# rare-resilience-ai/Osteosarcoma_DiffusionModel

Measured on AMD Instinct MI355X. Metric: synthetic patients/sec (full T-step reverse sample), higher is better.
Workload: dtype f32; 1 GPU; reverse sampling of conditional patients, T=1000, D=2000 (50 mut + 1900 expr + 50 pathway), hidden [256,512,256], 3 scenario conditions (BASELINE config 3); patients_per_gpu=100000, T=1000, parallelism=patients sharded over 1 GPU(s), no collective, sampler=chain, chunk_rows=65536, streams=2, graph=True

## Files before the change

### osteosarcoma_diffusionmodel_amd/csrc/chain.h

```cpp
#pragma once
#include "gemm_glds.h"
#include "epilogues.h"
#include "xpose.h"
#include "launch.h"

namespace osd {

constexpr int CHAIN_MAX_LAYERS = 24;
enum : int { CK_INPUT = 0, CK_GN32 = 1, CK_GN64 = 2, CK_POST = 3 };
enum : unsigned { CHAIN_OK = 0, CHAIN_TIMEOUT = 1, CHAIN_ABORT = 2 };

struct ChainLayer {
  const float* A; int lda;
  int K, K0;
  int F;
  int in0, ld0, in1, ld1;
  int out, ldo;
  int kind;
  const float* bias; const float* gamma; const float* beta;
};

struct ChainArgs {
  ChainLayer L[CHAIN_MAX_LAYERS];
  int n_layers;
  float* ws; long long ws_stride;
  float* x; int D;
  int n, n_tiles;
  int t_first, n_steps;
  unsigned base_done;
  const float* cproj; int ldc;
  const float* temb; int ldt;
  const float* coef;
  const float* z; int ldzz; long long z_step_stride; int z_t_first;
  uint64_t seed; uint32_t row_offset;
  float* mut_mask; int mutation_dim;
  unsigned* progress;
  unsigned* status;
  unsigned* queue;
  unsigned* cu_arrivals;
  int stagger;
  unsigned long long spin_budget;
  unsigned long long* stamps;
};

typedef __attribute__((address_space(1))) unsigned gu32;

__device__ __forceinline__ unsigned ld_relaxed_agent(const unsigned* p) {
  return __hip_atomic_load(p, __ATOMIC_RELAXED, __HIP_MEMORY_SCOPE_AGENT);
}
__device__ __forceinline__ void st_relaxed_agent(unsigned* p, unsigned v) {
  __hip_atomic_store(p, v, __ATOMIC_RELAXED, __HIP_MEMORY_SCOPE_AGENT);
}

__device__ __forceinline__ bool chain_wait(const unsigned* word, unsigned want, unsigned* status, unsigned long long budget, int lane) {
  if ((unsigned)__builtin_amdgcn_readfirstlane((int)ld_relaxed_agent(word)) >= want) return true;
  const unsigned long long t0 = __builtin_amdgcn_s_memrealtime();
  for (;;) {
    __builtin_amdgcn_s_sleep(32);
    if ((unsigned)__builtin_amdgcn_readfirstlane((int)ld_relaxed_agent(word)) >= want) return true;
    if ((unsigned)__builtin_amdgcn_readfirstlane((int)ld_relaxed_agent(status)) != CHAIN_OK) return false;
    if (__builtin_amdgcn_s_memrealtime() - t0 > budget) {
      if (lane == 0) st_relaxed_agent(status, CHAIN_TIMEOUT);
      return false;
    }
  }
}

constexpr int CHAIN_PRM_FLOATS = 512;

template <int NPB>
struct XposeRowsOut {
  const WaveXpose<NPB>& xp; float* out; int ldo;
  __device__ __forceinline__ void put(int fb, int pb, int q, int l31, int h, float4 v) const { (void)fb; xp.put(pb, q, l31, h, v); }
  __device__ __forceinline__ void flush(int fb, int lane) const { xp.template store_rows<false>(out + 32 * fb, ldo, lane, 0, 0); }
};
template <int NPB>
struct XposeRowsIn {
  const WaveXpose<NPB>& xp; const float* src; int ld;
  __device__ __forceinline__ void load(int fb, int lane) const { xp.template load_rows<false>(src + 32 * fb, ld, lane, 0, 0); }
  __device__ __forceinline__ float4 get(int fb, int pb, int q, int l31, int h) const { (void)fb; return xp.get(pb, q, l31, h); }
};

template <int GW, int NFB, int NPB, int PS, class Out>
__device__ __forceinline__ void chain_gn_silu(f32x16 (&acc)[NFB][NPB], const float* __restrict__ prm, int fl, const Out& o, int lane,
                                              unsigned long long* ts = nullptr) {
  static_assert(GW >= 8 && NFB * 32 >= GW, "wave must own whole groups");
  constexpr int RPG = GW / 2;
  constexpr int NG = NFB * 16 / RPG;
  const int l31 = lane & 31, h = lane >> 5;
#pragma unroll
  for (int fb = 0; fb < NFB; ++fb)
#pragma unroll
    for (int q = 0; q < 4; ++q) {
      const float4 bv = *reinterpret_cast<const float4*>(prm + fl + 32 * fb + 8 * q + 4 * h);
#pragma unroll
      for (int pb = 0; pb < NPB; ++pb) {
        acc[fb][pb][4 * q] += bv.x; acc[fb][pb][4 * q + 1] += bv.y;
        acc[fb][pb][4 * q + 2] += bv.z; acc[fb][pb][4 * q + 3] += bv.w;
      }
    }
  if (ts) { asm volatile("s_waitcnt vmcnt(0) lgkmcnt(0)" ::: "memory"); ts[0] = __builtin_amdgcn_s_memtime(); }
  float mean[NPB][NG], rstd[NPB][NG];
#pragma unroll
  for (int pb = 0; pb < NPB; ++pb)
#pragma unroll
    for (int g = 0; g < NG; ++g) {
      float s = 0.f;
#pragma unroll
      for (int j = 0; j < RPG; ++j) { const int Li = g * RPG + j; s += acc[Li / 16][pb][Li % 16]; }
      s += swap_halves(s);
      const float m = s * (1.0f / GW);
      float qs = 0.f;
#pragma unroll
      for (int j = 0; j < RPG; ++j) { const int Li = g * RPG + j; const float d = acc[Li / 16][pb][Li % 16] - m; qs = fmaf(d, d, qs); }
      qs += swap_halves(qs);
      mean[pb][g] = m;
      rstd[pb][g] = 1.0f / sqrtf(qs * (1.0f / GW) + GN_EPS);
    }
  if (ts) { asm volatile("s_nop 0" ::: "memory"); ts[1] = __builtin_amdgcn_s_memtime(); ts[2] = ts[1]; }
#pragma unroll
  for (int fb = 0; fb < NFB; ++fb) {
#pragma unroll
    for (int q = 0; q < 4; ++q) {
      const int f = fl + 32 * fb + 8 * q + 4 * h;
      const float4 gv = *reinterpret_cast<const float4*>(prm + PS + f);
      const float4 bev = *reinterpret_cast<const float4*>(prm + 2 * PS + f);
      const int g = (fb * 16 + 4 * q) / RPG;
#pragma unroll
      for (int pb = 0; pb < NPB; ++pb) {
        const float m = mean[pb][g], r = rstd[pb][g];
        float4 y;
        y.x = silu_f(fmaf((acc[fb][pb][4 * q] - m) * r, gv.x, bev.x));
        y.y = silu_f(fmaf((acc[fb][pb][4 * q + 1] - m) * r, gv.y, bev.y));
        y.z = silu_f(fmaf((acc[fb][pb][4 * q + 2] - m) * r, gv.z, bev.z));
        y.w = silu_f(fmaf((acc[fb][pb][4 * q + 3] - m) * r, gv.w, bev.w));
        o.put(fb, pb, q, l31, h, y);
      }
    }
    o.flush(fb, lane);
  }
}

template <int NFB, int NPB, int PS, class In, class Out>
__device__ __forceinline__ void chain_input(f32x16 (&acc)[NFB][NPB], const float* __restrict__ prm, int fl, const In& in, const Out& o, int lane) {
  const int l31 = lane & 31, h = lane >> 5;
#pragma unroll
  for (int fb = 0; fb < NFB; ++fb) {
    in.load(fb, lane);
#pragma unroll
    for (int q = 0; q < 4; ++q) {
      const int f = fl + 32 * fb + 8 * q + 4 * h;
      const float4 bv = *reinterpret_cast<const float4*>(prm + f);
      const float4 tv = *reinterpret_cast<const float4*>(prm + PS + f);
#pragma unroll
      for (int pb = 0; pb < NPB; ++pb) {
        const float4 cv = in.get(fb, pb, q, l31, h);
        float4 v;
        v.x = ((acc[fb][pb][4 * q] + bv.x) + tv.x) + cv.x;
        v.y = ((acc[fb][pb][4 * q + 1] + bv.y) + tv.y) + cv.y;
        v.z = ((acc[fb][pb][4 * q + 2] + bv.z) + tv.z) + cv.z;
        v.w = ((acc[fb][pb][4 * q + 3] + bv.w) + tv.w) + cv.w;
        o.put(fb, pb, q, l31, h, v);
      }
    }
    o.flush(fb, lane);
  }
}

#ifndef OSD_EXP
#define OSD_EXP 0
#endif
template <int NFB, int NPB, bool PRE = false, bool GUARD = true>
__device__ __forceinline__ void chain_posterior(f32x16 (&acc)[NFB][NPB], const float* __restrict__ prm, int fl, float* __restrict__ x, int ldx,
                                                int prow, int pcol, float cA, float cB, float cC, int t, const float* __restrict__ zrow, int ldzz,
                                                uint64_t seed, uint32_t row_id0, int f_glob, float* __restrict__ mut_mask, int mutation_dim,
                                                const WaveXpose<NPB>& xp, int lane, float4 (*pre)[4 * NPB] = nullptr) {
  const int l31 = lane & 31, h = lane >> 5;
  if (prow <= 0) return;
  const bool do_mask = t == 0 && mut_mask != nullptr;
#pragma unroll
  for (int fb = 0; fb < NFB; ++fb) {
    const int cols = pcol - 32 * fb;
    if (GUARD && cols <= 0) break;
    if constexpr (PRE) {
      if (!(OSD_EXP & 2)) {
        xp.commit_rows(*pre, lane);
        if (fb + 1 < NFB && cols - 32 > 0) xp.template issue_rows<GUARD>(*pre, x + 32 * (fb + 1), ldx, lane, prow, cols - 32);
      }
    } else {
      xp.template load_rows<GUARD>(x + 32 * fb, ldx, lane, prow, cols);
    }
#pragma unroll
    for (int pb = 0; pb < NPB; ++pb) {
      const int p = 32 * pb + l31;
      const int pc = (!GUARD || p < prow) ? p : prow - 1;
#pragma unroll
      for (int q = 0; q < 4; ++q) {
        const int fo = 32 * fb + 8 * q + 4 * h;
        const float4 bv = *reinterpret_cast<const float4*>(prm + fl + fo);
        const float e[4] = {acc[fb][pb][4 * q] + bv.x, acc[fb][pb][4 * q + 1] + bv.y, acc[fb][pb][4 * q + 2] + bv.z, acc[fb][pb][4 * q + 3] + bv.w};
        const float4 xq = xp.get(pb, q, l31, h);
        const float xv[4] = {xq.x, xq.y, xq.z, xq.w};
        float4 zz = make_float4(0.f, 0.f, 0.f, 0.f);
        if (t > 0 && cC != 0.f) {
          if (zrow) {
            const int fc = (!GUARD || fo < pcol - 4) ? fo : pcol - 4;
            zz = ldg4(zrow + (size_t)pc * ldzz + fc);
          } else if (!(OSD_EXP & 1)) {
            zz = randn4(seed, row_id0 + (uint32_t)p, (uint32_t)((f_glob + fo) >> 2), (uint32_t)t, TAG_POSTERIOR);
          }
        }
        const float zv[4] = {zz.x, zz.y, zz.z, zz.w};
        float o[4];
#pragma unroll
        for (int r = 0; r < 4; ++r) o[r] = fmaf(cA, xv[r], fmaf(cB, e[r], cC * zv[r]));
        if (do_mask && p < prow && fo < pcol && f_glob + fo < mutation_dim) {
          float* mrow = mut_mask + (size_t)p * mutation_dim;
#pragma unroll
          for (int r = 0; r < 4; ++r)
            if (f_glob + fo + r < mutation_dim) stg1(mrow + f_glob + fo + r, (o[r] > 0.5f) ? 1.0f : 0.0f);
        }
        xp.put(pb, q, l31, h, make_float4(o[0], o[1], o[2], o[3]));
      }
    }
    if (!(OSD_EXP & 4)) xp.template store_rows<GUARD>(x + 32 * fb, ldx, lane, prow, cols);
  }
}

#ifndef CHAIN_EPI_PRIO
#define CHAIN_EPI_PRIO 0
#endif
#ifndef CHAIN_BP
#define CHAIN_BP 128
#endif
#if CHAIN_BP == 128
typedef Tile<128, 128, 64, 64> ChainTile;
constexpr int CHAIN_WPS = 2;
#else
typedef Tile<128, 64, 64, 32> ChainTile;
constexpr int CHAIN_WPS = 3;
#endif
#ifdef OSD_DIAG
constexpr int CHAIN_KCNT = 12;
constexpr int CHAIN_STAMP_FLOATS = 2 * 4 * CHAIN_KCNT;
#else
constexpr int CHAIN_KCNT = 10;
constexpr int CHAIN_STAMP_FLOATS = 80;
#endif
constexpr int CHAIN_PRM_OFF = 2 * (ChainTile::BF * BK + ChainTile::BP * BK) + 4 + CHAIN_STAMP_FLOATS;
constexpr int CHAIN_LDS_BYTES = (CHAIN_PRM_OFF + 2 * CHAIN_PRM_FLOATS) * 4;
static_assert(CHAIN_PRM_OFF % 4 == 0, "parameter blocks are read as float4");

template <bool STAMP>
__global__ __launch_bounds__(NTHREADS, CHAIN_WPS) void chain_kernel(const ChainArgs* __restrict__ gp) {
  const ChainArgs& a = *gp;
  typedef ChainTile T;
  typedef GldsTile<T> G;
  static_assert(T::BF == 128 && T::BP % 32 == 0, "staging below assumes a 128-row weight image");
  constexpr int NW = NTHREADS / 64;
  constexpr int NPW = 16 / NW;
  constexpr int NPWB = T::BP / 8 / NW;
  constexpr int PROWS = 8 * NW;
  constexpr unsigned PBYTES = 1024u * NW;
  extern __shared__ __attribute__((aligned(16))) float smem[];
  float* As0 = smem;
  float* As1 = smem + G::A_ELEMS;
  float* Bs0 = smem + 2 * G::A_ELEMS;
  float* Bs1 = smem + 2 * G::A_ELEMS + G::B_ELEMS;
  volatile int& s_flag = *reinterpret_cast<volatile int*>(smem + 2 * (G::A_ELEMS + G::B_ELEMS));

  const int tid = threadIdx.x;
  const int lane = tid & 63;
  const int wave = __builtin_amdgcn_readfirstlane(tid >> 6);
  const int wf = (wave / T::NWP) * T::WF;
  const int wp = (wave % T::NWP) * T::WP;

  float* const ws = a.ws + (long long)blockIdx.x * a.ws_stride;
  WaveXpose<T::NPB> xp;
  {
    const int xo = wave * (T::NPB * 1024);
    xp.buf = xo < G::A_ELEMS ? As1 + xo : Bs1 + (xo - G::A_ELEMS);
  }
  float* const prm_base = smem + CHAIN_PRM_OFF;
  int pcur = 0;

  if (a.cu_arrivals && a.stagger > 0) {
    if (wave == 0) {
      const unsigned hw = __builtin_amdgcn_s_getreg(0xF804);
      const unsigned xcc = __builtin_amdgcn_s_getreg(0xF814) & 7;
      const unsigned key = (xcc << 8) | ((hw >> 8) & 0xFF);
      unsigned r = 0;
      if (lane == 0) r = atomicAdd(a.cu_arrivals + key, 1u);
      s_flag = __builtin_amdgcn_readfirstlane((int)(r & 1u));
    }
    __syncthreads();
    const int late = __builtin_amdgcn_readfirstlane(s_flag);
    __syncthreads();
    if (late) {
      const unsigned long long t0 = __builtin_amdgcn_s_memtime();
      while (__builtin_amdgcn_s_memtime() - t0 < (unsigned long long)a.stagger) __builtin_amdgcn_s_sleep(16);
    }
  }

  unsigned long long c_dep = 0, c_pro = 0, c_k = 0, c_epi = 0, c_units = 0;
  unsigned long long* const kcnt = reinterpret_cast<unsigned long long*>(smem + 2 * (G::A_ELEMS + G::B_ELEMS) + 4);
  if constexpr (STAMP) {
    if (tid < 4 * CHAIN_KCNT) kcnt[tid] = 0;
    __syncthreads();
  }
  const unsigned long long c_start = STAMP ? __builtin_amdgcn_s_memtime() : 0;
  const long long n_units = (long long)a.n_tiles * a.n_steps;
  int c_iter = 0;
  (void)c_iter;
  for (;;) {
    const unsigned long long td0 = STAMP ? __builtin_amdgcn_s_memtime() : 0;
#ifdef CHAIN_STATIC_UNITS
    static_assert(true, "");
    const long long u = (long long)blockIdx.x + (long long)c_iter * gridDim.x;
    ++c_iter;
#else
    if (wave == 0) {
      unsigned nu = 0;
      if (lane == 0) nu = atomicAdd(a.queue, 1u);
      s_flag = __builtin_amdgcn_readfirstlane((int)nu);
    }
    __syncthreads();
    const long long u = (unsigned)__builtin_amdgcn_readfirstlane(s_flag);
    __syncthreads();
#endif
    if (u >= n_units) break;
    const int tile = (int)(u % a.n_tiles);
    const int si = (int)(u / a.n_tiles);
    const int t = a.t_first - si;
    const int p0 = tile * T::BP;
    const int P = (a.n - p0 < T::BP) ? a.n - p0 : T::BP;

    if (wave == 0) {
      bool ok = (unsigned)__builtin_amdgcn_readfirstlane((int)ld_relaxed_agent(a.status)) == CHAIN_OK;
      if (ok && si > 0) {
        ok = chain_wait(a.progress + tile, a.base_done + (unsigned)si, a.status, a.spin_budget, lane);
        if (ok) __builtin_amdgcn_fence(__ATOMIC_ACQUIRE, "agent");
      }
      s_flag = ok ? 1 : 0;
      asm volatile("s_waitcnt vmcnt(0) lgkmcnt(0)" ::: "memory");
    }
    __syncthreads();
    const int go = __builtin_amdgcn_readfirstlane(s_flag);
    if (!go) return;
    if constexpr (STAMP) { c_dep += __builtin_amdgcn_s_memtime() - td0; ++c_units; }

    auto first_stage = [&](const ChainLayer& Lr, int f0n, bool do_a, bool do_b, int pb) {
      struct { const float* A; int lda, F, in0, ld0, K0, K; } Ln{Lr.A, Lr.lda, Lr.F, Lr.in0, Lr.ld0, Lr.K0, Lr.K};
      if (do_a && wave < 2) {
        const int kind = Lr.kind;
        const float* src = Lr.bias;
        if (wave == 1) src = Lr.beta;
        else if (lane >= 32) src = kind == CK_INPUT ? a.temb + (size_t)t * a.ldt : (kind == CK_POST ? Lr.bias : Lr.gamma);
        if (wave == 0 || (kind != CK_INPUT && kind != CK_POST)) {
          int f = f0n + 4 * (lane & 31);
          f = f < Ln.F - 4 ? f : Ln.F - 4;
          glds16(src + f, __builtin_amdgcn_readfirstlane(lds_addr(prm_base + pb * CHAIN_PRM_FLOATS) + (unsigned)wave * 1024u));
        }
      }
      const float* const xrows = a.x + (size_t)p0 * a.D;
      int ln = lane;
      asm volatile("" : "+v"(ln));
      const int r0 = wave * 8 + (ln >> 3);
      const int k4 = 4 * ((ln & 7) ^ ((r0 >> 1) & 7));
      const unsigned la = __builtin_amdgcn_readfirstlane(lds_addr(As0) + (unsigned)wave * 1024u);
      const unsigned lb = __builtin_amdgcn_readfirstlane(lds_addr(Bs0) + (unsigned)wave * 1024u);
      if (do_a) {
#pragma unroll
        for (int j = 0; j < NPW; ++j) {
          int rg = f0n + r0 + PROWS * j;
          rg = rg < Ln.F ? rg : Ln.F - 1;
          glds16(Ln.A + (size_t)rg * Ln.lda + k4, __builtin_amdgcn_readfirstlane(la + (unsigned)j * PBYTES));
        }
      }
      if (do_b) {
        const bool from_x = Ln.in0 < 0;
        const float* bb = from_x ? xrows : ws + Ln.in0;
        const int rows = from_x ? P : T::BP;
        const int kend = Ln.K0 < Ln.K ? Ln.K0 : Ln.K;
        const int k = k4 < kend - 4 ? k4 : kend - 4;
#pragma unroll
        for (int j = 0; j < NPWB; ++j) {
          int rg = r0 + PROWS * j;
          rg = rg < rows ? rg : rows - 1;
          glds16(bb + (size_t)rg * Ln.ld0 + k, __builtin_amdgcn_readfirstlane(lb + (unsigned)j * PBYTES));
        }
      }
    };
    unsigned long long tt0 = STAMP ? __builtin_amdgcn_s_memtime() : 0;
    first_stage(a.L[0], 0, true, true, pcur);
    asm volatile("s_waitcnt vmcnt(0)" ::: "memory");
    __syncthreads();

    for (int l = 0; l < a.n_layers; ++l) {
      const ChainLayer& L = a.L[l];
      const gfloat_ptr LA = uniform_ptr(L.A);
      const int Llda = L.lda, LK0 = L.K0, Lld0 = L.ld0, Lld1 = L.ld1;
      const int F = L.F, K = L.K;
      const float* const B0g = (L.in0 < 0) ? a.x + (size_t)p0 * a.D : ws + L.in0;
      const float* const B1g = ws + L.in1;
      const gfloat_ptr B0 = uniform_ptr(B0g), B1 = uniform_ptr(B1g);
      const int rowsB = (L.in0 < 0) ? P : T::BP;
      const int nk = (K + BK - 1) / BK;
      const int nft = (F + T::BF - 1) / T::BF;
      for (int ft = 0; ft < nft; ++ft) {
        const int f0 = ft * T::BF;
        int ln = lane;
        asm volatile("" : "+v"(ln));
        const int l31 = ln & 31, h = ln >> 5;
        int st_row[NPW], st_k4[NPW];
#pragma unroll
        for (int j = 0; j < NPW; ++j) {
          st_row[j] = (j * NW + wave) * 8 + (ln >> 3);
          st_k4[j] = 4 * ((ln & 7) ^ ((st_row[j] >> 1) & 7));
        }
        int a_rd[T::NFB], a_sw[T::NFB], b_rd[T::NPB], b_sw[T::NPB];
#pragma unroll
        for (int fb = 0; fb < T::NFB; ++fb) { const int R = wf + 32 * fb + l31; a_rd[fb] = R * BK; a_sw[fb] = h ^ ((R >> 1) & 7); }
#pragma unroll
        for (int pb = 0; pb < T::NPB; ++pb) { const int R = wp + 32 * pb + l31; b_rd[pb] = R * BK; b_sw[pb] = h ^ ((R >> 1) & 7); }
        unsigned offA[NPW], offB[NPWB];
#pragma unroll
        for (int j = 0; j < NPW; ++j) {
          int rg = f0 + st_row[j];
          rg = rg < F ? rg : F - 1;
          offA[j] = (unsigned)(rg * Llda + st_k4[j]) * 4u;
        }
#pragma unroll
        for (int j = 0; j < NPWB; ++j) {
          int rb = st_row[j];
          rb = rb < rowsB ? rb : rowsB - 1;
          offB[j] = (unsigned)(rb * Lld0 + st_k4[j]) * 4u;
        }
        int b_panel = 0;
        auto b_offsets_for = [&](int k0) {
          const int want = k0 < LK0 ? 0 : 1;
          if (want != b_panel) {
            b_panel = want;
            const int ld = want ? Lld1 : Lld0;
#pragma unroll
            for (int j = 0; j < NPWB; ++j) {
              int rb = st_row[j];
              rb = rb < rowsB ? rb : rowsB - 1;
              offB[j] = (unsigned)(rb * ld + st_k4[j]) * 4u;
            }
          }
        };
        struct StageCtx { gfloat_ptr sa, sb; unsigned la, lb; int k0; bool tail; };
        auto stage_begin = [&](int k0, float* As, float* Bs) {
          b_offsets_for(k0);
          const bool first = k0 < LK0;
          const int kend = first ? (LK0 < K ? LK0 : K) : K - LK0;
          const int kl = first ? k0 : k0 - LK0;
          StageCtx c;
          c.sa = LA + __builtin_amdgcn_readfirstlane(k0);
          c.sb = (first ? B0 : B1) + __builtin_amdgcn_readfirstlane(kl);
          c.la = __builtin_amdgcn_readfirstlane(lds_addr(As) + (unsigned)wave * 1024u);
          c.lb = __builtin_amdgcn_readfirstlane(lds_addr(Bs) + (unsigned)wave * 1024u);
          c.k0 = k0;
          c.tail = kl + BK > kend;
          return c;
        };
        auto piece = [&](const StageCtx& c, int j) {
          if (j < NPW) glds16s(c.sa, offA[j], __builtin_amdgcn_readfirstlane(c.la + (unsigned)j * PBYTES));
          else glds16s(c.sb, offB[j - NPW], __builtin_amdgcn_readfirstlane(c.lb + (unsigned)(j - NPW) * PBYTES));
        };
        auto stage_tail = [&](const StageCtx& c) {
#pragma unroll
          for (int j = 0; j < NPW; ++j) piece(c, j);
          const bool first = c.k0 < LK0;
          const int kend = first ? (LK0 < K ? LK0 : K) : K - LK0;
          const int kl = first ? c.k0 : c.k0 - LK0;
          const float* bb = first ? B0g : B1g;
          const int ld = first ? Lld0 : Lld1;
#pragma unroll
          for (int jb = 0; jb < NPWB; ++jb) {
            int k = kl + st_k4[jb];
            k = k < kend - 4 ? k : kend - 4;
            int rg = st_row[jb];
            rg = rg < rowsB ? rg : rowsB - 1;
            glds16(bb + (size_t)rg * ld + k, __builtin_amdgcn_readfirstlane(c.lb + (unsigned)jb * PBYTES));
          }
        };
        const unsigned long long tt1 = STAMP ? __builtin_amdgcn_s_memtime() : 0;

        unsigned long long c_kw = 0, c_kb = 0;
        (void)c_kw; (void)c_kb;
        f32x16 acc[T::NFB][T::NPB];
#pragma unroll
        for (int i = 0; i < T::NFB; ++i)
#pragma unroll
          for (int j = 0; j < T::NPB; ++j)
#pragma unroll
            for (int r = 0; r < 16; ++r) acc[i][j][r] = 0.f;

        float fa0[T::NFB][4], fb0[T::NPB][4], fa1[T::NFB][4], fb1[T::NPB][4];
        auto frags = [&](const float* Ac, const float* Bc, int i, float (&fa)[T::NFB][4], float (&fb)[T::NPB][4]) {
#pragma unroll
          for (int fb_ = 0; fb_ < T::NFB; ++fb_) {
            const float4 tq = *reinterpret_cast<const float4*>(&Ac[a_rd[fb_] + 4 * (a_sw[fb_] ^ (2 * i))]);
            fa[fb_][0] = tq.x; fa[fb_][1] = tq.y; fa[fb_][2] = tq.z; fa[fb_][3] = tq.w;
          }
#pragma unroll
          for (int pb = 0; pb < T::NPB; ++pb) {
            const float4 tq = *reinterpret_cast<const float4*>(&Bc[b_rd[pb] + 4 * (b_sw[pb] ^ (2 * i))]);
            fb[pb][0] = tq.x; fb[pb][1] = tq.y; fb[pb][2] = tq.z; fb[pb][3] = tq.w;
          }
        };
        auto quarter = [&](const float (&fa)[T::NFB][4], const float (&fb)[T::NPB][4]) {
#pragma unroll
          for (int e = 0; e < 4; ++e)
#pragma unroll
            for (int fb_ = 0; fb_ < T::NFB; ++fb_)
#pragma unroll
              for (int pb = 0; pb < T::NPB; ++pb)
                acc[fb_][pb] = __builtin_amdgcn_mfma_f32_32x32x2f32(fa[fb_][e], fb[pb][e], acc[fb_][pb], 0, 0, 0);
        };
        __builtin_amdgcn_sched_barrier(0);
        if (nk > 1) {
          const StageCtx c = stage_begin(BK, As1, Bs1);
          if (c.tail) stage_tail(c);
          else {
#pragma unroll
            for (int j = 0; j < NPW + NPWB; ++j) piece(c, j);
          }
        }
        frags(As0, Bs0, 0, fa0, fb0);
        __builtin_amdgcn_sched_barrier(0);
        for (int kt = 0; kt < nk; ++kt) {
          float* Ac = (kt & 1) ? As1 : As0;
          float* Bc = (kt & 1) ? Bs1 : Bs0;
          const float* An = (kt & 1) ? As0 : As1;
          const float* Bn = (kt & 1) ? Bs0 : Bs1;
          frags(Ac, Bc, 1, fa1, fb1);
          quarter(fa0, fb0);
          frags(Ac, Bc, 2, fa0, fb0);
          quarter(fa1, fb1);
          frags(Ac, Bc, 3, fa1, fb1);
          const bool ahead = kt + 2 < nk;
          StageCtx c{};
          if (ahead) c = stage_begin((kt + 2) * BK, Ac, Bc);
          const bool whole = ahead && !c.tail;
          quarter(fa0, fb0);
          __builtin_amdgcn_sched_barrier(0);
          const unsigned long long tw0 = STAMP ? __builtin_amdgcn_s_memtime() : 0;
          asm volatile("s_waitcnt vmcnt(0)" ::: "memory");
          const unsigned long long tw1 = STAMP ? __builtin_amdgcn_s_memtime() : 0;
          asm volatile("s_waitcnt lgkmcnt(0)" ::: "memory");
          __syncthreads();
          if constexpr (STAMP) { const unsigned long long tw2 = __builtin_amdgcn_s_memtime(); c_kw += tw1 - tw0; c_kb += tw2 - tw1; }
          __builtin_amdgcn_sched_barrier(0);
          if (ahead && c.tail) stage_tail(c);
          if (whole) {
#pragma unroll
            for (int j = 0; j < NPW + NPWB; ++j) piece(c, j);
          }
          if (kt + 1 < nk) frags(An, Bn, 0, fa0, fb0);
          __builtin_amdgcn_sched_barrier(0);
          quarter(fa1, fb1);
        }

        const unsigned long long tt2 = STAMP ? __builtin_amdgcn_s_memtime() : 0;
        const bool same_layer = ft + 1 < nft;
        const bool has_next = same_layer || l + 1 < a.n_layers;
        const int ln_next = same_layer ? l : l + 1;
        const int f0_next = same_layer ? f0 + T::BF : 0;
        const bool early_b = same_layer;
        if (has_next) first_stage(a.L[ln_next], f0_next, true, early_b, pcur ^ 1);
        const int fw = f0 + wf;
        const float* const prm = prm_base + pcur * CHAIN_PRM_FLOATS;
        pcur ^= 1;
        if (CHAIN_EPI_PRIO) __builtin_amdgcn_s_setprio(CHAIN_EPI_PRIO);
        const ChainArgs* ep = gp;
        asm volatile("" : "+s"(ep));
        const ChainArgs& e = *ep;
        unsigned long long ets[3] = {0, 0, 0};
        if (L.kind == CK_GN64) {
          const XposeRowsOut<T::NPB> o{xp, ws + L.out + (size_t)wp * L.ldo + fw, L.ldo};
          chain_gn_silu<64, T::NFB, T::NPB, 128>(acc, prm, wf, o, lane, STAMP ? ets : nullptr);
        } else if (L.kind == CK_GN32) {
          const XposeRowsOut<T::NPB> o{xp, ws + L.out + (size_t)wp * L.ldo + fw, L.ldo};
          chain_gn_silu<32, T::NFB, T::NPB, 128>(acc, prm, wf, o, lane, STAMP ? ets : nullptr);
        } else if (L.kind == CK_INPUT) {
          const XposeRowsIn<T::NPB> ci{xp, e.cproj + (size_t)(p0 + wp) * e.ldc + fw, e.ldc};
          const XposeRowsOut<T::NPB> o{xp, ws + L.out + (size_t)wp * L.ldo + fw, L.ldo};
          chain_input<T::NFB, T::NPB, 128>(acc, prm, wf, ci, o, lane);
        } else {
          const float* c = e.coef + 4 * t;
          const float cA = c[0], cB = c[1], cC = c[2];
          const float* zrow = e.z ? e.z + (long long)(e.z_t_first - t) * e.z_step_stride + (size_t)(p0 + wp) * e.ldzz + fw : nullptr;
          float* const mm = e.mut_mask ? e.mut_mask + (size_t)(p0 + wp) * e.mutation_dim : nullptr;
          chain_posterior<T::NFB, T::NPB>(acc, prm, wf, e.x + (size_t)(p0 + wp) * e.D + fw, e.D, P - wp, F - fw, cA, cB, cC, t, zrow, e.ldzz,
                                          e.seed, e.row_offset + (uint32_t)(p0 + wp), fw, mm, e.mutation_dim, xp, lane);
        }
        if (CHAIN_EPI_PRIO) __builtin_amdgcn_s_setprio(0);
        unsigned long long tt3 = 0, te1 = 0, te2 = 0, te3 = 0, te4 = 0;
        if constexpr (STAMP) te1 = __builtin_amdgcn_s_memtime();
        if (early_b) {
          if constexpr (STAMP) tt3 = __builtin_amdgcn_s_memtime();
          static_assert(4 * T::NFB * T::NPB == 16 || 4 * T::NFB * T::NPB == 8, "counted wait below is written for 16 or 8 stores");
          if (L.kind == CK_POST) asm volatile("s_waitcnt vmcnt(0)" ::: "memory");
          else if (4 * T::NFB * T::NPB == 16) asm volatile("s_waitcnt vmcnt(16)" ::: "memory");
          else asm volatile("s_waitcnt vmcnt(8)" ::: "memory");
          if constexpr (STAMP) te2 = __builtin_amdgcn_s_memtime();
          __syncthreads();
          if constexpr (STAMP) te3 = te4 = __builtin_amdgcn_s_memtime();
        } else {
          asm volatile("s_waitcnt vmcnt(0)" ::: "memory");
          if constexpr (STAMP) te2 = __builtin_amdgcn_s_memtime();
          __syncthreads();
          if constexpr (STAMP) tt3 = te3 = __builtin_amdgcn_s_memtime();
          if (has_next) {
            first_stage(a.L[ln_next], 0, false, true, 0);
            asm volatile("s_waitcnt vmcnt(0)" ::: "memory");
            __syncthreads();
          }
          if constexpr (STAMP) te4 = __builtin_amdgcn_s_memtime();
        }
        if constexpr (STAMP) {
          c_pro += tt1 - tt0; c_k += tt2 - tt1; c_epi += tt3 - tt2;
          tt0 = tt3;
          if (tid == 0) {
            unsigned long long* kc = kcnt + CHAIN_KCNT * L.kind;
            kc[0] += tt2 - tt1; kc[1] += te1 - tt2; kc[2] += te2 - te1; kc[3] += te3 - te2; kc[4] += te4 - te3; kc[5] += 1;
            if constexpr (CHAIN_KCNT >= 12) { kc[10] += c_kw; kc[11] += c_kb; }
            if (ets[0]) { kc[6] += ets[0] - tt2; kc[7] += ets[1] - ets[0]; kc[8] += ets[2] - ets[1]; kc[9] += te1 - ets[2]; }
          }
        }
      }
    }

    if (wave == 0) {
      __builtin_amdgcn_fence(__ATOMIC_RELEASE, "agent");
      asm volatile("s_waitcnt vmcnt(0)" ::: "memory");
      if (lane == 0) st_relaxed_agent(a.progress + tile, a.base_done + (unsigned)si + 1u);
    }
  }
  if (STAMP && a.stamps && tid == 0) {
    unsigned long long* o = a.stamps + (size_t)blockIdx.x * 64;
    o[0] = c_dep; o[1] = c_pro; o[2] = c_k; o[3] = c_epi; o[4] = __builtin_amdgcn_s_memtime() - c_start; o[5] = c_units;
    o[6] = __builtin_amdgcn_s_getreg(0xF804);
    o[7] = __builtin_amdgcn_s_getreg(0xF814) & 7;
    for (int i = 0; i < 4 * CHAIN_KCNT; ++i) o[8 + i] = kcnt[i];
  }
}

}
```

### osteosarcoma_diffusionmodel_amd/csrc/gemm_glds.h

```cpp
#pragma once
#include "gemm.h"

namespace osd {

typedef __attribute__((address_space(3))) void* lds_ptr_t;
typedef const __attribute__((address_space(1))) void* glb_ptr_t;

__device__ __forceinline__ void glds16(const float* gsrc, unsigned lds_dst) {
  unsigned keep;
  asm volatile(
      "s_mov_b32 %0, m0\n\t"
      "s_mov_b32 m0, %2\n\t"
      "s_nop 0\n\t"
      "global_load_lds_dwordx4 %1, off\n\t"
      "s_mov_b32 m0, %0"
      : "=&s"(keep)
      : "v"(gsrc), "s"(lds_dst)
      : "memory");
}
typedef const __attribute__((address_space(1))) float* gfloat_ptr;
__device__ __forceinline__ gfloat_ptr uniform_ptr(const float* p) {
  const gfloat_ptr q = (gfloat_ptr)p;
  const unsigned long long v = reinterpret_cast<unsigned long long>(q);
  const unsigned lo = __builtin_amdgcn_readfirstlane((unsigned)v), hi = __builtin_amdgcn_readfirstlane((unsigned)(v >> 32));
  return reinterpret_cast<gfloat_ptr>(((unsigned long long)hi << 32) | lo);
}
__device__ __forceinline__ void glds16s(gfloat_ptr sbase, unsigned voff, unsigned lds_dst) {
  unsigned keep;
  asm volatile(
      "s_mov_b32 %0, m0\n\t"
      "s_mov_b32 m0, %3\n\t"
      "s_nop 4\n\t"
      "global_load_lds_dwordx4 %1, %2\n\t"
      "s_mov_b32 m0, %0"
      : "=&s"(keep)
      : "v"(voff), "s"(sbase), "s"(lds_dst)
      : "memory");
}
__device__ __forceinline__ unsigned lds_addr(const float* p) {
  return (unsigned)(uintptr_t)(__attribute__((address_space(3))) const void*)p;
}

template <class T>
struct GldsTile {
  static constexpr int A_ELEMS = T::BF * BK;
  static constexpr int B_ELEMS = T::BP * BK;
  static constexpr int LDS_BYTES = 2 * (A_ELEMS + B_ELEMS) * 4;
  static constexpr int NA = T::BF / 32;
  static constexpr int NB = T::BP / 32;
};

template <class T, class Epi, int NG = 1>
__global__ __launch_bounds__(NTHREADS * NG, NG == 1 ? 2 : 1) void gemm_glds_kernel(GemmArgs g, typename Epi::Args ea) {
  typedef GldsTile<T> G;
  static_assert(NG == 1 || NG == 2, "one or two wave groups");
  extern __shared__ __attribute__((aligned(16))) float smem_all[];
  const int grp = NG == 1 ? 0 : __builtin_amdgcn_readfirstlane((int)(threadIdx.x >> 8));
  float* const smem = smem_all + grp * (G::LDS_BYTES / 4);
  float* As0 = smem;
  float* As1 = smem + G::A_ELEMS;
  float* Bs0 = smem + 2 * G::A_ELEMS;
  float* Bs1 = smem + 2 * G::A_ELEMS + G::B_ELEMS;

  const int nft = (g.F + T::BF - 1) / T::BF;
  const int npt = (g.P + T::BP - 1) / T::BP;
  const int b = blockIdx.x;
  const int idx = b >> 3;
  const int ft = idx % nft;
  int pt, pstride;
  if (g.persist) {
    const int per_xcd = gridDim.x >> 3;
    pt = idx / nft + (per_xcd / nft) * (b & 7);
    pstride = gridDim.x / nft;
  } else {
    pt = (idx / nft) * 8 + (b & 7);
    pstride = npt;
  }
  if (pt >= npt) return;
  if (g.tri && ft > pt) return;
  const int f0 = ft * T::BF;

  const int tid = threadIdx.x & (NTHREADS - 1);
  const int lane = tid & 63;
  const int wave = __builtin_amdgcn_readfirstlane(tid >> 6);
  unsigned long long st0 = 0, st1 = 0, st2 = 0;
  if (g.stamps) st0 = __builtin_amdgcn_s_memtime();
  const int wf = (wave / T::NWP) * T::WF;
  const int wp = (wave % T::NWP) * T::WP;
  const int l31 = lane & 31, h = lane >> 5;

  const auto pre = Epi::template prefetch<T::NFB, true>(ea, f0 + wf, lane, g.F);

  int a_off[G::NA], a_k4[G::NA];
  int b_k4[G::NB], b_lrow[G::NB];
#pragma unroll
  for (int j = 0; j < G::NA; ++j) {
    const int row = (j * 4 + wave) * 8 + (lane >> 3);
    int rg = f0 + row;
    rg = rg < g.F ? rg : g.F - 1;
    a_k4[j] = 4 * ((lane & 7) ^ ((row >> 1) & 7));
    a_off[j] = rg * g.lda + a_k4[j];
  }
#pragma unroll
  for (int j = 0; j < G::NB; ++j) {
    const int row = (j * 4 + wave) * 8 + (lane >> 3);
    b_lrow[j] = row;
    b_k4[j] = 4 * ((lane & 7) ^ ((row >> 1) & 7));
  }
  struct StageCtx { unsigned la, lb; const float* bbase; int bld, bk, bkend, ak, p0; };
  auto stage_begin = [&](int k0, int p0, float* As, float* Bs) {
    StageCtx c;
    c.la = __builtin_amdgcn_readfirstlane(lds_addr(As) + (unsigned)wave * 1024u);
    c.lb = __builtin_amdgcn_readfirstlane(lds_addr(Bs) + (unsigned)wave * 1024u);
    const bool first = k0 < g.K0;
    c.bbase = first ? g.B0 : g.B1;
    c.bld = first ? g.ldb0 : g.ldb1;
    c.bk = first ? k0 : k0 - g.K0;
    c.bkend = first ? (g.K0 < g.K ? g.K0 : g.K) : g.K - g.K0;
    c.ak = k0;
    c.p0 = p0;
    return c;
  };
  auto stage_piece = [&](const StageCtx& c, int j) {
    if (j < G::NA) {
      int adj = 0;
      if (g.a_kmax > 0) {
        const int k = c.ak + a_k4[j];
        adj = k < g.a_kmax - 4 ? 0 : g.a_kmax - 4 - k;
      }
      glds16(g.A + (size_t)(a_off[j] + c.ak + adj), __builtin_amdgcn_readfirstlane(c.la + (unsigned)j * 4096u));
    } else {
      const int jb = j - G::NA;
      int k = c.bk + b_k4[jb];
      k = k < c.bkend - 4 ? k : c.bkend - 4;
      int rg = c.p0 + b_lrow[jb];
      rg = rg < g.P ? rg : g.P - 1;
      glds16(c.bbase + (size_t)rg * c.bld + k, __builtin_amdgcn_readfirstlane(c.lb + (unsigned)jb * 4096u));
    }
  };
  constexpr int NPIECE = G::NA + G::NB;

  int a_rd[T::NFB], a_sw[T::NFB], b_rd[T::NPB], b_sw[T::NPB];
#pragma unroll
  for (int fb = 0; fb < T::NFB; ++fb) { const int R = wf + 32 * fb + l31; a_rd[fb] = R * BK; a_sw[fb] = h ^ ((R >> 1) & 7); }
#pragma unroll
  for (int pb = 0; pb < T::NPB; ++pb) { const int R = wp + 32 * pb + l31; b_rd[pb] = R * BK; b_sw[pb] = h ^ ((R >> 1) & 7); }

  f32x16 acc[T::NFB][T::NPB];

  auto compute = [&](const float* As, const float* Bs, int i, const StageCtx& sc, bool do_stage) {
    float a[T::NFB][4], bb[T::NPB][4];
#pragma unroll
    for (int fb = 0; fb < T::NFB; ++fb) {
      const float4 t = *reinterpret_cast<const float4*>(&As[a_rd[fb] + 4 * (a_sw[fb] ^ (2 * i))]);
      a[fb][0] = t.x; a[fb][1] = t.y; a[fb][2] = t.z; a[fb][3] = t.w;
    }
#pragma unroll
    for (int pb = 0; pb < T::NPB; ++pb) {
      const float4 t = *reinterpret_cast<const float4*>(&Bs[b_rd[pb] + 4 * (b_sw[pb] ^ (2 * i))]);
      bb[pb][0] = t.x; bb[pb][1] = t.y; bb[pb][2] = t.z; bb[pb][3] = t.w;
    }
#pragma unroll
    for (int e = 0; e < 4; ++e) {
#pragma unroll
      for (int fb = 0; fb < T::NFB; ++fb)
#pragma unroll
        for (int pb = 0; pb < T::NPB; ++pb)
          acc[fb][pb] = __builtin_amdgcn_mfma_f32_32x32x2f32(a[fb][e], bb[pb][e], acc[fb][pb], 0, 0, 0);
      if (do_stage && i == 0) {
        __builtin_amdgcn_sched_barrier(0);
        if (2 * e < NPIECE) stage_piece(sc, 2 * e);
        if (2 * e + 1 < NPIECE) stage_piece(sc, 2 * e + 1);
        __builtin_amdgcn_sched_barrier(0);
      }
    }
  };

  const int nk_all = (g.K + BK - 1) / BK;
  const int nk = NG == 1 ? nk_all : (nk_all + 1) / 2;
  const int kbeg = grp ? nk : 0;
  const int kcnt = NG == 1 ? nk : (grp ? nk_all - nk : nk);
  {
    const StageCtx c0 = stage_begin(kbeg * BK, pt * T::BP, As0, Bs0);
#pragma unroll
    for (int j = 0; j < NPIECE; ++j) stage_piece(c0, j);
  }
  constexpr int FULL_TILE_STORES = T::NFB * T::NPB * 4;
  bool counted_wait = false;
  for (; pt < npt; pt += pstride) {
    const int p0 = pt * T::BP;
    if (counted_wait) {
      if constexpr (FULL_TILE_STORES == 16) asm volatile("s_waitcnt vmcnt(16)" ::: "memory");
      else if constexpr (FULL_TILE_STORES == 8) asm volatile("s_waitcnt vmcnt(8)" ::: "memory");
      else if constexpr (FULL_TILE_STORES == 4) asm volatile("s_waitcnt vmcnt(4)" ::: "memory");
      else asm volatile("s_waitcnt vmcnt(0)" ::: "memory");
    } else {
      asm volatile("s_waitcnt vmcnt(0)" ::: "memory");
    }
    __syncthreads();
    if (g.stamps && st1 == 0) st1 = __builtin_amdgcn_s_memtime();
#pragma unroll
    for (int i = 0; i < T::NFB; ++i)
#pragma unroll
      for (int j = 0; j < T::NPB; ++j)
#pragma unroll
        for (int r = 0; r < 16; ++r) acc[i][j][r] = 0.f;
    for (int kt = 0; kt < nk; ++kt) {
      float* Ac = (kt & 1) ? As1 : As0;
      float* Bc = (kt & 1) ? Bs1 : Bs0;
      const bool more = kt + 1 < kcnt;
      const StageCtx sc = stage_begin(more ? (kbeg + kt + 1) * BK : 0, p0, (kt & 1) ? As0 : As1, (kt & 1) ? Bs0 : Bs1);
      if (NG == 1 || kt < kcnt) {
        compute(Ac, Bc, 0, sc, more);
        compute(Ac, Bc, 1, sc, more);
        compute(Ac, Bc, 2, sc, more);
        compute(Ac, Bc, 3, sc, more);
      }
      asm volatile("s_waitcnt vmcnt(0)" ::: "memory");
      __syncthreads();
    }
    if (g.stamps && st2 == 0) st2 = __builtin_amdgcn_s_memtime();
    const int ptn = pt + pstride;
    if (ptn < npt) {
      const StageCtx cn = stage_begin(0, ptn * T::BP, As0, Bs0);
#pragma unroll
      for (int j = 0; j < NPIECE; ++j) stage_piece(cn, j);
    }
    if constexpr (NG == 2) {
      constexpr int NREG = T::NFB * T::NPB * 16;
      static_assert(4 * NREG * 64 * 4 <= G::LDS_BYTES, "accumulator hand-over must fit the group's staging buffers");
      float* const red = smem_all + G::LDS_BYTES / 4 + wave * (NREG * 64);
      if (grp == 1) {
#pragma unroll
        for (int i = 0; i < T::NFB; ++i)
#pragma unroll
          for (int j = 0; j < T::NPB; ++j)
#pragma unroll
            for (int r = 0; r < 16; ++r) red[((i * T::NPB + j) * 16 + r) * 64 + lane] = acc[i][j][r];
      }
      __syncthreads();
      if (grp == 1) return;
#pragma unroll
      for (int i = 0; i < T::NFB; ++i)
#pragma unroll
        for (int j = 0; j < T::NPB; ++j)
#pragma unroll
          for (int r = 0; r < 16; ++r) acc[i][j][r] += red[((i * T::NPB + j) * 16 + r) * 64 + lane];
    }
    counted_wait = Epi::COUNTED_STORES && (p0 + T::BP <= g.P) && (f0 + T::BF <= g.F);
    if constexpr (Epi::XBUF) {
      constexpr int XR = T::NPB * 1024;
      static_assert(G::A_ELEMS % XR == 0 && 4 * XR <= G::A_ELEMS + G::B_ELEMS, "transposer regions must tile the idle buffers");
      const int xo = wave * XR;
      float* const xb = xo < G::A_ELEMS ? As1 + xo : Bs1 + (xo - G::A_ELEMS);
      Epi::template apply<T::NFB, T::NPB, true>(acc, ea, pre, f0 + wf, p0 + wp, lane, g.F, g.P, xb);
    } else {
      Epi::template apply<T::NFB, T::NPB, true>(acc, ea, pre, f0 + wf, p0 + wp, lane, g.F, g.P);
    }
  }
  if (g.stamps) {
    asm volatile("s_waitcnt vmcnt(0)" ::: "memory");
    const unsigned long long st3 = __builtin_amdgcn_s_memtime();
    if (lane == 0) {
      unsigned long long* o = g.stamps + ((size_t)blockIdx.x * 4 + wave) * 4;
      o[0] = st0; o[1] = st1; o[2] = st2; o[3] = st3;
    }
  }
}

}
```

Measured before the change: 22820 patients/s.

## Batch global-to-LDS staging into single asm blocks with immediate offsets and steady-state runs

Reorganises the chain kernel's K-loop staging so each wave loads contiguous LDS pieces, letting the pieces of one operand share a single m0 setup and differ only by immediate offsets in one inline-asm block. It adds a steady-state path that advances scalar base pointers instead of recomputing stage context per k-step, unrolls the loop by two with compile-time buffer parity, and precomputes LDS fragment read addresses. The aim is to cut scalar/VALU address overhead and m0 churn in the inner loop, at the cost of a new staging layout that must stay consistent with the fragment reads and a biased-pointer trick that relies on offset arithmetic.

Result: no change. 22920 patients/s (median of 6 runs) (+0.4%).

```diff
diff --git a/osteosarcoma_diffusionmodel_amd/csrc/chain.h b/osteosarcoma_diffusionmodel_amd/csrc/chain.h
--- a/osteosarcoma_diffusionmodel_amd/csrc/chain.h
+++ b/osteosarcoma_diffusionmodel_amd/csrc/chain.h
@@ -1,4 +1,5 @@
 #pragma once
+#include <type_traits>
 #include "gemm_glds.h"
 #include "epilogues.h"
 #include "xpose.h"
@@ -260,8 +261,8 @@
   constexpr int NW = NTHREADS / 64;
   constexpr int NPW = 16 / NW;
   constexpr int NPWB = T::BP / 8 / NW;
-  constexpr int PROWS = 8 * NW;
-  constexpr unsigned PBYTES = 1024u * NW;
+  constexpr unsigned PBYTES = 1024u;
+  static_assert(NPW == 4 && (NPWB == 4 || NPWB == 2), "glds16_stage is written for these piece counts");
   extern __shared__ __attribute__((aligned(16))) float smem[];
   float* As0 = smem;
   float* As1 = smem + G::A_ELEMS;
@@ -274,6 +275,8 @@
   const int wave = __builtin_amdgcn_readfirstlane(tid >> 6);
   const int wf = (wave / T::NWP) * T::WF;
   const int wp = (wave % T::NWP) * T::WP;
+  auto st_row_of = [&](int np, int j, int ln) { return (np * wave + j) * 8 + (ln >> 3); };
+  auto st_k4_of = [](int row, int ln) { return 4 * ((ln & 7) ^ ((row >> 1) & 7)); };
 
   float* const ws = a.ws + (long long)blockIdx.x * a.ws_stride;
   WaveXpose<T::NPB> xp;
@@ -309,7 +312,7 @@
     __syncthreads();
   }
   const unsigned long long c_start = STAMP ? __builtin_amdgcn_s_memtime() : 0;
-  const long long n_units = (long long)a.n_tiles * a.n_steps;
+  const long long n_units = (long long)__builtin_amdgcn_readfirstlane(a.n_tiles) * __builtin_amdgcn_readfirstlane(a.n_steps);
   int c_iter = 0;
   (void)c_iter;
   for (;;) {
@@ -365,16 +368,15 @@
       const float* const xrows = a.x + (size_t)p0 * a.D;
       int ln = lane;
       asm volatile("" : "+v"(ln));
-      const int r0 = wave * 8 + (ln >> 3);
-      const int k4 = 4 * ((ln & 7) ^ ((r0 >> 1) & 7));
-      const unsigned la = __builtin_amdgcn_readfirstlane(lds_addr(As0) + (unsigned)wave * 1024u);
-      const unsigned lb = __builtin_amdgcn_readfirstlane(lds_addr(Bs0) + (unsigned)wave * 1024u);
+      const unsigned la = __builtin_amdgcn_readfirstlane(lds_addr(As0) + (unsigned)wave * (NPW * PBYTES));
+      const unsigned lb = __builtin_amdgcn_readfirstlane(lds_addr(Bs0) + (unsigned)wave * (NPWB * PBYTES));
       if (do_a) {
 #pragma unroll
         for (int j = 0; j < NPW; ++j) {
-          int rg = f0n + r0 + PROWS * j;
+          const int r = st_row_of(NPW, j, ln);
+          int rg = f0n + r;
           rg = rg < Ln.F ? rg : Ln.F - 1;
-          glds16(Ln.A + (size_t)rg * Ln.lda + k4, __builtin_amdgcn_readfirstlane(la + (unsigned)j * PBYTES));
+          glds16(Ln.A + (size_t)rg * Ln.lda + st_k4_of(r, ln), __builtin_amdgcn_readfirstlane(la + (unsigned)j * PBYTES));
         }
       }
       if (do_b) {
@@ -382,11 +384,12 @@
         const float* bb = from_x ? xrows : ws + Ln.in0;
         const int rows = from_x ? P : T::BP;
         const int kend = Ln.K0 < Ln.K ? Ln.K0 : Ln.K;
-        const int k = k4 < kend - 4 ? k4 : kend - 4;
 #pragma unroll
         for (int j = 0; j < NPWB; ++j) {
-          int rg = r0 + PROWS * j;
-          rg = rg < rows ? rg : rows - 1;
+          const int r = st_row_of(NPWB, j, ln);
+          const int k4 = st_k4_of(r, ln);
+          const int k = k4 < kend - 4 ? k4 : kend - 4;
+          const int rg = r < rows ? r : rows - 1;
           glds16(bb + (size_t)rg * Ln.ld0 + k, __builtin_amdgcn_readfirstlane(lb + (unsigned)j * PBYTES));
         }
       }
@@ -406,83 +409,80 @@
       const gfloat_ptr B0 = uniform_ptr(B0g), B1 = uniform_ptr(B1g);
       const int rowsB = (L.in0 < 0) ? P : T::BP;
       const int nk = (K + BK - 1) / BK;
+      const int kp0 = LK0 < K ? LK0 : K;
+      const int n0 = (kp0 + BK - 1) / BK, w0 = kp0 / BK, w1 = n0 + (K - kp0) / BK;
+      const gfloat_ptr LAb = glds_biased(LA), B0b = glds_biased(B0), B1b = glds_biased(B1);
       const int nft = (F + T::BF - 1) / T::BF;
       for (int ft = 0; ft < nft; ++ft) {
         const int f0 = ft * T::BF;
         int ln = lane;
         asm volatile("" : "+v"(ln));
         const int l31 = ln & 31, h = ln >> 5;
-        int st_row[NPW], st_k4[NPW];
+        unsigned fr_a[4], fr_b[4];
+#pragma unroll
+        for (int i = 0; i < 4; ++i) {
+          const int Ra = wf + l31, Rb = wp + l31;
+          fr_a[i] = lds_addr(As0) + (unsigned)(Ra * BK + 4 * ((h ^ ((Ra >> 1) & 7)) ^ (2 * i))) * 4u;
+          fr_b[i] = lds_addr(Bs0) + (unsigned)(Rb * BK + 4 * ((h ^ ((Rb >> 1) & 7)) ^ (2 * i))) * 4u;
+          asm volatile("" : "+v"(fr_a[i]), "+v"(fr_b[i]));
+        }
+        unsigned offA[NPW], offB[NPWB];
 #pragma unroll
         for (int j = 0; j < NPW; ++j) {
-          st_row[j] = (j * NW + wave) * 8 + (ln >> 3);
-          st_k4[j] = 4 * ((ln & 7) ^ ((st_row[j] >> 1) & 7));
-        }
-        int a_rd[T::NFB], a_sw[T::NFB], b_rd[T::NPB], b_sw[T::NPB];
-#pragma unroll
-        for (int fb = 0; fb < T::NFB; ++fb) { const int R = wf + 32 * fb + l31; a_rd[fb] = R * BK; a_sw[fb] = h ^ ((R >> 1) & 7); }
-#pragma unroll
-        for (int pb = 0; pb < T::NPB; ++pb) { const int R = wp + 32 * pb + l31; b_rd[pb] = R * BK; b_sw[pb] = h ^ ((R >> 1) & 7); }
-        unsigned offA[NPW], offB[NPWB];
-#pragma unroll
-        for (int j = 0; j < NPW; ++j) {
-          int rg = f0 + st_row[j];
+          const int r = st_row_of(NPW, j, ln);
+          int rg = f0 + r;
           rg = rg < F ? rg : F - 1;
-          offA[j] = (unsigned)(rg * Llda + st_k4[j]) * 4u;
-        }
-#pragma unroll
-        for (int j = 0; j < NPWB; ++j) {
-          int rb = st_row[j];
-          rb = rb < rowsB ? rb : rowsB - 1;
-          offB[j] = (unsigned)(rb * Lld0 + st_k4[j]) * 4u;
-        }
+          offA[j] = (unsigned)(rg * Llda + st_k4_of(r, ln)) * 4u + (GLDS_OFF_BIAS - 1024u * j);
+        }
+        auto b_offsets = [&](int ld) {
+#pragma unroll
+          for (int j = 0; j < NPWB; ++j) {
+            const int r = st_row_of(NPWB, j, ln);
+            const int rb = r < rowsB ? r : rowsB - 1;
+            offB[j] = (unsigned)(rb * ld + st_k4_of(r, ln)) * 4u + (GLDS_OFF_BIAS - 1024u * j);
+          }
+        };
+        b_offsets(Lld0);
         int b_panel = 0;
         auto b_offsets_for = [&](int k0) {
           const int want = k0 < LK0 ? 0 : 1;
           if (want != b_panel) {
             b_panel = want;
-            const int ld = want ? Lld1 : Lld0;
-#pragma unroll
-            for (int j = 0; j < NPWB; ++j) {
-              int rb = st_row[j];
-              rb = rb < rowsB ? rb : rowsB - 1;
-              offB[j] = (unsigned)(rb * ld + st_k4[j]) * 4u;
-            }
-          }
-        };
+            b_offsets(want ? Lld1 : Lld0);
+          }
+        };
+        const unsigned la0 = __builtin_amdgcn_readfirstlane(lds_addr(As0) + (unsigned)wave * (NPW * PBYTES));
+        const unsigned lb0 = __builtin_amdgcn_readfirstlane(lds_addr(Bs0) + (unsigned)wave * (NPWB * PBYTES));
+        constexpr unsigned A_BUF = G::A_ELEMS * 4u, B_BUF = G::B_ELEMS * 4u;
         struct StageCtx { gfloat_ptr sa, sb; unsigned la, lb; int k0; bool tail; };
-        auto stage_begin = [&](int k0, float* As, float* Bs) {
+        auto stage_begin = [&](int k0, int par) {
           b_offsets_for(k0);
           const bool first = k0 < LK0;
-          const int kend = first ? (LK0 < K ? LK0 : K) : K - LK0;
+          const int kend = first ? kp0 : K - LK0;
           const int kl = first ? k0 : k0 - LK0;
           StageCtx c;
-          c.sa = LA + __builtin_amdgcn_readfirstlane(k0);
-          c.sb = (first ? B0 : B1) + __builtin_amdgcn_readfirstlane(kl);
-          c.la = __builtin_amdgcn_readfirstlane(lds_addr(As) + (unsigned)wave * 1024u);
-          c.lb = __builtin_amdgcn_readfirstlane(lds_addr(Bs) + (unsigned)wave * 1024u);
+          c.sa = LAb + __builtin_amdgcn_readfirstlane(k0);
+          c.sb = (first ? B0b : B1b) + __builtin_amdgcn_readfirstlane(kl);
+          c.la = la0 + (unsigned)par * A_BUF;
+          c.lb = lb0 + (unsigned)par * B_BUF;
           c.k0 = k0;
           c.tail = kl + BK > kend;
           return c;
         };
-        auto piece = [&](const StageCtx& c, int j) {
-          if (j < NPW) glds16s(c.sa, offA[j], __builtin_amdgcn_readfirstlane(c.la + (unsigned)j * PBYTES));
-          else glds16s(c.sb, offB[j - NPW], __builtin_amdgcn_readfirstlane(c.lb + (unsigned)(j - NPW) * PBYTES));
-        };
+        auto stage_whole = [&](const StageCtx& c) { glds16_stage<NPWB>(c.sa, offA, c.la, c.sb, offB, c.lb); };
         auto stage_tail = [&](const StageCtx& c) {
-#pragma unroll
-          for (int j = 0; j < NPW; ++j) piece(c, j);
+          glds16_quad<NPW>(c.sa, offA, c.la);
           const bool first = c.k0 < LK0;
-          const int kend = first ? (LK0 < K ? LK0 : K) : K - LK0;
+          const int kend = first ? kp0 : K - LK0;
           const int kl = first ? c.k0 : c.k0 - LK0;
           const float* bb = first ? B0g : B1g;
           const int ld = first ? Lld0 : Lld1;
 #pragma unroll
           for (int jb = 0; jb < NPWB; ++jb) {
-            int k = kl + st_k4[jb];
+            const int r = st_row_of(NPWB, jb, ln);
+            int k = kl + st_k4_of(r, ln);
             k = k < kend - 4 ? k : kend - 4;
-            int rg = st_row[jb];
-            rg = rg < rowsB ? rg : rowsB - 1;
+            const int rg = r < rowsB ? r : rowsB - 1;
             glds16(bb + (size_t)rg * ld + k, __builtin_amdgcn_readfirstlane(c.lb + (unsigned)jb * PBYTES));
           }
         };
@@ -499,15 +499,15 @@
             for (int r = 0; r < 16; ++r) acc[i][j][r] = 0.f;
 
         float fa0[T::NFB][4], fb0[T::NPB][4], fa1[T::NFB][4], fb1[T::NPB][4];
-        auto frags = [&](const float* Ac, const float* Bc, int i, float (&fa)[T::NFB][4], float (&fb)[T::NPB][4]) {
+        auto frags = [&](int par, int i, float (&fa)[T::NFB][4], float (&fb)[T::NPB][4]) {
 #pragma unroll
           for (int fb_ = 0; fb_ < T::NFB; ++fb_) {
-            const float4 tq = *reinterpret_cast<const float4*>(&Ac[a_rd[fb_] + 4 * (a_sw[fb_] ^ (2 * i))]);
+            const f32x4v tq = lds_read16(fr_a[i] + (unsigned)par * A_BUF + (unsigned)fb_ * (32u * BK * 4u));
             fa[fb_][0] = tq.x; fa[fb_][1] = tq.y; fa[fb_][2] = tq.z; fa[fb_][3] = tq.w;
           }
 #pragma unroll
           for (int pb = 0; pb < T::NPB; ++pb) {
-            const float4 tq = *reinterpret_cast<const float4*>(&Bc[b_rd[pb] + 4 * (b_sw[pb] ^ (2 * i))]);
+            const f32x4v tq = lds_read16(fr_b[i] + (unsigned)par * B_BUF + (unsigned)pb * (32u * BK * 4u));
             fb[pb][0] = tq.x; fb[pb][1] = tq.y; fb[pb][2] = tq.z; fb[pb][3] = tq.w;
           }
         };
@@ -522,29 +522,37 @@
         };
         __builtin_amdgcn_sched_barrier(0);
         if (nk > 1) {
-          const StageCtx c = stage_begin(BK, As1, Bs1);
+          const StageCtx c = stage_begin(BK, 1);
           if (c.tail) stage_tail(c);
-          else {
-#pragma unroll
-            for (int j = 0; j < NPW + NPWB; ++j) piece(c, j);
-          }
-        }
-        frags(As0, Bs0, 0, fa0, fb0);
+          else stage_whole(c);
+        }
+        frags(0, 0, fa0, fb0);
         __builtin_amdgcn_sched_barrier(0);
-        for (int kt = 0; kt < nk; ++kt) {
-          float* Ac = (kt & 1) ? As1 : As0;
-          float* Bc = (kt & 1) ? Bs1 : Bs0;
-          const float* An = (kt & 1) ? As0 : As1;
-          const float* Bn = (kt & 1) ? Bs0 : Bs1;
-          frags(Ac, Bc, 1, fa1, fb1);
+        gfloat_ptr sa, sb;
+        int run_end;
+        auto run_from = [&](int s) {
+          run_end = b_panel ? w1 : w0;
+          sa = LAb + __builtin_amdgcn_readfirstlane(s * BK);
+          sb = (b_panel ? B1b : B0b) + __builtin_amdgcn_readfirstlane((b_panel ? s - n0 : s) * BK);
+        };
+        run_from(2);
+        auto step = [&](auto par_c, int kt) {
+          constexpr int PAR = decltype(par_c)::value;
+          frags(PAR, 1, fa1, fb1);
           quarter(fa0, fb0);
-          frags(Ac, Bc, 2, fa0, fb0);
+          frags(PAR, 2, fa0, fb0);
           quarter(fa1, fb1);
-          frags(Ac, Bc, 3, fa1, fb1);
-          const bool ahead = kt + 2 < nk;
+          frags(PAR, 3, fa1, fb1);
+          const bool steady = kt + 2 < run_end;
+          const bool ahead = !steady && kt + 2 < nk;
           StageCtx c{};
-          if (ahead) c = stage_begin((kt + 2) * BK, Ac, Bc);
-          const bool whole = ahead && !c.tail;
+          if (ahead) {
+            const int pan = b_panel;
+            int k0 = (kt + 2) * BK;
+            asm volatile("" : "+s"(k0));
+            c = stage_begin(k0, PAR);
+            if (b_panel != pan) run_from(kt + 3);
+          }
           quarter(fa0, fb0);
           __builtin_amdgcn_sched_barrier(0);
           const unsigned long long tw0 = STAMP ? __builtin_amdgcn_s_memtime() : 0;
@@ -554,15 +562,23 @@
           __syncthreads();
           if constexpr (STAMP) { const unsigned long long tw2 = __builtin_amdgcn_s_memtime(); c_kw += tw1 - tw0; c_kb += tw2 - tw1; }
           __builtin_amdgcn_sched_barrier(0);
-          if (ahead && c.tail) stage_tail(c);
-          if (whole) {
-#pragma unroll
-            for (int j = 0; j < NPW + NPWB; ++j) piece(c, j);
-          }
-          if (kt + 1 < nk) frags(An, Bn, 0, fa0, fb0);
+          if (steady) {
+            glds16_stage<NPWB>(sa, offA, la0 + PAR * A_BUF, sb, offB, lb0 + PAR * B_BUF);
+            sa += BK;
+            sb += BK;
+          } else if (ahead) {
+            if (c.tail) stage_tail(c);
+            else stage_whole(c);
+          }
+          if (kt + 1 < nk) frags(PAR ^ 1, 0, fa0, fb0);
           __builtin_amdgcn_sched_barrier(0);
           quarter(fa1, fb1);
-        }
+        };
+        for (int kt = 0; kt + 1 < nk; kt += 2) {
+          step(std::integral_constant<int, 0>{}, kt);
+          step(std::integral_constant<int, 1>{}, kt + 1);
+        }
+        if (nk & 1) step(std::integral_constant<int, 0>{}, nk - 1);
 
         const unsigned long long tt2 = STAMP ? __builtin_amdgcn_s_memtime() : 0;
         const bool same_layer = ft + 1 < nft;
diff --git a/osteosarcoma_diffusionmodel_amd/csrc/gemm_glds.h b/osteosarcoma_diffusionmodel_amd/csrc/gemm_glds.h
--- a/osteosarcoma_diffusionmodel_amd/csrc/gemm_glds.h
+++ b/osteosarcoma_diffusionmodel_amd/csrc/gemm_glds.h
@@ -36,6 +36,59 @@
       : "=&s"(keep)
       : "v"(voff), "s"(sbase), "s"(lds_dst)
       : "memory");
+}
+constexpr unsigned GLDS_OFF_BIAS = 3072;
+__device__ __forceinline__ gfloat_ptr glds_biased(gfloat_ptr p) { return p - GLDS_OFF_BIAS / 4; }
+#define OSD_GLDS4(V, S)                                      \
+  "global_load_lds_dwordx4 %[" #V "0], %[" #S "]\n\t"             \
+  "global_load_lds_dwordx4 %[" #V "1], %[" #S "] offset:1024\n\t" \
+  "global_load_lds_dwordx4 %[" #V "2], %[" #S "] offset:2048\n\t" \
+  "global_load_lds_dwordx4 %[" #V "3], %[" #S "] offset:3072\n\t"
+#define OSD_GLDS2(V, S)                                      \
+  "global_load_lds_dwordx4 %[" #V "0], %[" #S "]\n\t"             \
+  "global_load_lds_dwordx4 %[" #V "1], %[" #S "] offset:1024\n\t"
+template <int NP>
+__device__ __forceinline__ void glds16_quad(gfloat_ptr sbase, const unsigned (&voff)[NP], unsigned lds_dst) {
+  static_assert(NP == 4 || NP == 2, "pieces per wave and operand");
+  unsigned keep;
+  if constexpr (NP == 4) {
+    asm volatile("s_nop 4\n\ts_mov_b32 %[k], m0\n\ts_mov_b32 m0, %[l]\n\ts_nop 0\n\t" OSD_GLDS4(a, s) "s_mov_b32 m0, %[k]"
+                 : [k] "=&s"(keep)
+                 : [a0] "v"(voff[0]), [a1] "v"(voff[1]), [a2] "v"(voff[2]), [a3] "v"(voff[3]), [s] "s"(sbase), [l] "s"(lds_dst)
+                 : "memory");
+  } else {
+    asm volatile("s_nop 4\n\ts_mov_b32 %[k], m0\n\ts_mov_b32 m0, %[l]\n\ts_nop 0\n\t" OSD_GLDS2(a, s) "s_mov_b32 m0, %[k]"
+                 : [k] "=&s"(keep)
+                 : [a0] "v"(voff[0]), [a1] "v"(voff[1]), [s] "s"(sbase), [l] "s"(lds_dst)
+                 : "memory");
+  }
+}
+template <int NB>
+__device__ __forceinline__ void glds16_stage(gfloat_ptr sa, const unsigned (&va)[4], unsigned la, gfloat_ptr sb, const unsigned (&vb)[NB],
+                                             unsigned lb) {
+  static_assert(NB == 4 || NB == 2, "pieces per wave and operand");
+  unsigned keep;
+  if constexpr (NB == 4) {
+    asm volatile("s_nop 4\n\ts_mov_b32 %[k], m0\n\ts_mov_b32 m0, %[la]\n\ts_nop 0\n\t" OSD_GLDS4(a, sa)
+                 "s_mov_b32 m0, %[lb]\n\ts_nop 0\n\t" OSD_GLDS4(b, sb) "s_mov_b32 m0, %[k]"
+                 : [k] "=&s"(keep)
+                 : [a0] "v"(va[0]), [a1] "v"(va[1]), [a2] "v"(va[2]), [a3] "v"(va[3]), [sa] "s"(sa), [la] "s"(la),
+                   [b0] "v"(vb[0]), [b1] "v"(vb[1]), [b2] "v"(vb[2]), [b3] "v"(vb[3]), [sb] "s"(sb), [lb] "s"(lb)
+                 : "memory");
+  } else {
+    asm volatile("s_nop 4\n\ts_mov_b32 %[k], m0\n\ts_mov_b32 m0, %[la]\n\ts_nop 0\n\t" OSD_GLDS4(a, sa)
+                 "s_mov_b32 m0, %[lb]\n\ts_nop 0\n\t" OSD_GLDS2(b, sb) "s_mov_b32 m0, %[k]"
+                 : [k] "=&s"(keep)
+                 : [a0] "v"(va[0]), [a1] "v"(va[1]), [a2] "v"(va[2]), [a3] "v"(va[3]), [sa] "s"(sa), [la] "s"(la),
+                   [b0] "v"(vb[0]), [b1] "v"(vb[1]), [sb] "s"(sb), [lb] "s"(lb)
+                 : "memory");
+  }
+}
+#undef OSD_GLDS4
+#undef OSD_GLDS2
+typedef float f32x4v __attribute__((ext_vector_type(4)));
+__device__ __forceinline__ f32x4v lds_read16(unsigned addr) {
+  return *reinterpret_cast<const __attribute__((address_space(3))) f32x4v*>((uintptr_t)addr);
 }
 __device__ __forceinline__ unsigned lds_addr(const float* p) {
   return (unsigned)(uintptr_t)(__attribute__((address_space(3))) const void*)p;
```
